# DUBSON0/iterative-closest-point-avmi

Measured on AMD Instinct MI355X. Metric: icp_iterations_per_sec, higher is better.
Workload: dtype f64

## Files before the change

iterative-closest-point-avmi_amd/csrc/prep.hip:

```cpp
#include "prep_common.hpp"

namespace icpmi {

#ifndef PREP_AXIS_STEP
#define PREP_AXIS_STEP 4
#endif
#ifndef ICPMI_PREP_WPS
#define ICPMI_PREP_WPS 6
#endif
constexpr int PREP_THREADS = 512;
constexpr int PREP_MAXW = PREP_THREADS / ICPMI_WAVE;
constexpr int PREP_MAX_POINTS = 4096;

constexpr float PREP_POLAR_Q = 6.283185307179586f / 2097152.0f;
__device__ __forceinline__ uint32_t prep_polar_key21(double x, double y) {
    const float t = (atan2f((float)y, (float)x) + 3.14159265f) * (2097152.0f / 6.283185307179586f);
    const int k = (int)t;
    return (uint32_t)(k < 0 ? 0 : (k > 2097151 ? 2097151 : k));
}
__device__ __forceinline__ float prep_polar_image(uint32_t k21) { return (float)k21 * PREP_POLAR_Q - 3.14159265f; }

template <int E>
__device__ __forceinline__ void prep_sort_polar32(const double* __restrict__ P, int M, uint64_t* keys, uint32_t* rows) {
    uint32_t v[E];
#pragma unroll
    for (int e = 0; e < E; ++e) {
        const int i = e * PREP_THREADS + (int)threadIdx.x;
        v[e] = i < M ? (prep_polar_key21(P[2 * i], P[2 * i + 1]) << 11) | (uint32_t)i : 0xffffffffu;
    }
    bitonic_sort_regs_fixed<uint32_t, E, PREP_THREADS>(v, reinterpret_cast<uint32_t*>(keys));
    __syncthreads();
#pragma unroll
    for (int e = 0; e < E; ++e) {
        const int i = (int)threadIdx.x * E + e;
        rows[i] = v[e] == 0xffffffffu ? 0xffffffffu : (v[e] & 0x7ffu);
        keys[i] = v[e] == 0xffffffffu ? ~0ull : f64_sortable((double)prep_polar_image(v[e] >> 11));
    }
    __syncthreads();
}

template <int E>
__device__ __forceinline__ void prep_sort_regs(const double* __restrict__ P, int M, int dir, uint64_t* by_row, uint64_t* keys,
                                               uint32_t* rows) {
    if (dir == SWEEP_POLAR) { prep_sort_polar32<E>(P, M, keys, rows); return; }
    constexpr uint64_t ROW_MASK = 0x7ff;
    uint64_t v[E];
#pragma unroll
    for (int e = 0; e < E; ++e) {
        const int i = (int)threadIdx.x * E + e;
        const uint64_t k = i < M ? f64_sortable(proj(dir, P[2 * i], P[2 * i + 1])) : ~0ull;
        by_row[i] = k;
        v[e] = i < M ? ((k & ~ROW_MASK) | (uint64_t)i) : ~0ull;
    }
    bitonic_sort_regs_fixed<uint64_t, E, PREP_THREADS>(v, keys);
    int bad = 0;
#pragma unroll
    for (int e = 0; e < E; ++e) {
        const int i = (int)threadIdx.x * E + e;
        const uint32_t r = v[e] == ~0ull ? 0xffffffffu : (uint32_t)(v[e] & ROW_MASK);
        rows[i] = r;
        keys[i] = r == 0xffffffffu ? ~0ull : by_row[r];
    }
    __syncthreads();
#pragma unroll
    for (int e = 0; e < E; ++e) {
        const int i = (int)threadIdx.x * E + e;
        if (i + 1 < M && (keys[i] > keys[i + 1] || (keys[i] == keys[i + 1] && rows[i] > rows[i + 1]))) bad = 1;
    }
    if (__syncthreads_or(bad)) {
        if (threadIdx.x == 0)
            for (int i = 1; i < M; ++i) {
                const uint64_t k = keys[i];
                const uint32_t r = rows[i];
                int j = i - 1;
                while (j >= 0 && (keys[j] > k || (keys[j] == k && rows[j] > r))) { keys[j + 1] = keys[j]; rows[j + 1] = rows[j]; --j; }
                keys[j + 1] = k; rows[j + 1] = r;
            }
        __syncthreads();
    }
}

template <int KK, bool GRID>
__global__ __launch_bounds__(PREP_THREADS, (KK <= 13 ? ICPMI_PREP_WPS : (KK <= 16 ? 4 : 2))) void prep_targets_kernel(
    const double* __restrict__ pts, const int32_t* __restrict__ off, const int32_t* __restrict__ cnt,
    const int32_t* __restrict__ cloud_ids, int k, double2* __restrict__ g_sxy, double2* __restrict__ g_snrm,
    int32_t* __restrict__ g_sorig, float* __restrict__ g_skey, int32_t* __restrict__ g_dir, double* __restrict__ out_normals,
    int lds_points, int split, int polar) {
    extern __shared__ __attribute__((aligned(16))) unsigned char dyn[];
    __shared__ double dsc[8 * PREP_MAXW];
    __shared__ int hist[6 * PREP_BINS];
    const int ci = blockIdx.x / split, part = blockIdx.x % split;
    const int c = cloud_ids ? cloud_ids[ci] : ci;
    const int M = cnt ? cnt[c] : off[c + 1] - off[c];
    if (off[c + 1] - off[c] > PREP_MAX_POINTS) return;
    if (M <= 0 || M > lds_points) { if (threadIdx.x == 0) g_dir[c] = -1; return; }
    const double* P = pts + (size_t)off[c] * 2;
    int npad = 64;
    while (npad < M) npad <<= 1;
    double2* sxy = reinterpret_cast<double2*>(dyn);
    int32_t* sorig = reinterpret_cast<int32_t*>(dyn + (size_t)lds_points * 16);
    float* sth = reinterpret_cast<float*>(dyn + (size_t)lds_points * 20);
    const size_t scratch_at = GRID ? (size_t)lds_points * 24 : 0;
    const bool reg_sort = npad <= 4 * PREP_THREADS;
    const int nsort = reg_sort ? max(npad, PREP_THREADS) : npad;
    uint64_t* by_row = reinterpret_cast<uint64_t*>(dyn + scratch_at);
    uint64_t* keys = reinterpret_cast<uint64_t*>(dyn + scratch_at + (reg_sort ? (size_t)nsort * 8 : 0));
    uint32_t* rows = reinterpret_cast<uint32_t*>(reinterpret_cast<unsigned char*>(keys) + (size_t)nsort * 8);

    double bounds[4];
    const int dir = choose_axis<PREP_THREADS>(P, M, dsc, hist, bounds, polar, (!GRID && M >= 512) ? PREP_AXIS_STEP : 1);
    if (reg_sort) {
        if (nsort == PREP_THREADS) prep_sort_regs<1>(P, M, dir, by_row, keys, rows);
        else if (nsort == 2 * PREP_THREADS) prep_sort_regs<2>(P, M, dir, by_row, keys, rows);
        else prep_sort_regs<4>(P, M, dir, by_row, keys, rows);
    } else {
        for (int i = threadIdx.x; i < npad; i += PREP_THREADS) {
            keys[i] = i < M ? f64_sortable(dir == SWEEP_POLAR ? polar_key(P[2 * i], P[2 * i + 1]) : proj(dir, P[2 * i], P[2 * i + 1])) : ~0ull;
            rows[i] = i < M ? (uint32_t)i : 0xffffffffu;
        }
        __syncthreads();
        bitonic_sort_pairs(keys, rows, npad);
    }
    double2* o_sxy = g_sxy + off[c];
    int32_t* o_sorig = g_sorig + off[c];
    float* o_skey = g_skey + off[c];
    int my_row[PREP_MAX_POINTS / PREP_THREADS];
    float my_key[PREP_MAX_POINTS / PREP_THREADS];
#pragma unroll
    for (int u = 0; u < PREP_MAX_POINTS / PREP_THREADS; ++u) {
        const int i = u * PREP_THREADS + (int)threadIdx.x;
        my_row[u] = i < M ? (int)rows[i] : 0;
        my_key[u] = i < M ? (float)f64_unsortable(keys[i]) : 0.0f;
    }
    __syncthreads();
#pragma unroll
    for (int u = 0; u < PREP_MAX_POINTS / PREP_THREADS; ++u) {
        const int i = u * PREP_THREADS + (int)threadIdx.x;
        if (i < M) {
            const int row = my_row[u];
            const double2 p = make_double2(P[2 * row], P[2 * row + 1]);
            sxy[i] = p; sorig[i] = row;
            if (KK > 0 && !GRID && dir == SWEEP_POLAR) sth[i] = my_key[u];
            if (part == 0) { o_sxy[i] = p; o_sorig[i] = row; o_skey[i] = my_key[u]; }
        }
    }
    if (threadIdx.x == 0 && part == 0) g_dir[c] = dir;
    __syncthreads();
    if constexpr (KK > 0) {
        const int kc = min(k, M - 1);
        const int kk = kc + 1;
        double2* o_snrm = g_snrm + off[c];
        double* o_rows = out_normals ? out_normals + (size_t)off[c] * 2 : nullptr;
        const int per = (M + split - 1) / split;
        if constexpr (GRID) {
            const int cells_cap = min(4096, 2 * npad);
            uint32_t* cell_end = reinterpret_cast<uint32_t*>(dyn + scratch_at);
            uint16_t* cell_pts = reinterpret_cast<uint16_t*>(cell_end + cells_cap);
            const PrepGrid grid = prep_grid_build(sxy, M, bounds, kk, cell_end, cell_pts, cells_cap, hist);
            prep_normals_grid<KK>(sxy, sorig, M, min(M, part * per), min(M, (part + 1) * per), kk, grid, o_snrm, o_rows);
        } else {
            if (dir == SWEEP_POLAR) prep_normals_polar<KK>(sxy, sorig, sth, M, min(M, part * per), min(M, (part + 1) * per), kk, o_snrm, o_rows);
            else prep_normals<KK>(sxy, sorig, M, min(M, part * per), min(M, (part + 1) * per), dir, kk, o_snrm, o_rows);
        }
    }
}


constexpr int ANYK_THREADS = 256;
__device__ __forceinline__ int anyk_lower_bound(const double2* sxy, int M, int dir, double v) {
    int lo = 0, hi = M;
    while (lo < hi) {
        const int mid = (lo + hi) >> 1;
        const double2 c = sxy[mid];
        if (proj(dir, c.x, c.y) < v) lo = mid + 1; else hi = mid;
    }
    return lo;
}
__global__ __launch_bounds__(ANYK_THREADS) void normals_anyk_kernel(
    const int32_t* __restrict__ off, const int32_t* __restrict__ cnt, const int32_t* __restrict__ cloud_ids, int k,
    const double2* __restrict__ g_sxy, double2* __restrict__ g_snrm, const int32_t* __restrict__ g_sorig,
    const int32_t* __restrict__ g_dir, double* __restrict__ out_normals, int sel_cap) {
    extern __shared__ __attribute__((aligned(16))) unsigned char dyn[];
    int32_t* sel = reinterpret_cast<int32_t*>(dyn) + (size_t)wave_id() * sel_cap;
    const int c = cloud_ids ? cloud_ids[blockIdx.y] : blockIdx.y;
    const int M = cnt ? min(cnt[c], off[c + 1] - off[c]) : off[c + 1] - off[c];
    const int dir = g_dir[c];
    if (M <= 0 || dir < 0) return;
    const double2* sxy = g_sxy + off[c];
    const int32_t* sorig = g_sorig + off[c];
    double2* o_snrm = g_snrm + off[c];
    double* o_rows = out_normals ? out_normals + (size_t)off[c] * 2 : nullptr;
    const int kk = min(min(k, M - 1) + 1, sel_cap);
    const int lane = lane_id();
    const int waves = gridDim.x * (ANYK_THREADS / ICPMI_WAVE);
    for (int s = blockIdx.x * (ANYK_THREADS / ICPMI_WAVE) + wave_id(); s < M; s += waves) {
        const double2 q = sxy[s];
        int lo = 0, hi = M;
        if (dir < SWEEP_POLAR) {
            const int a0 = max(0, s - kk), a1 = min(M - 1, s + kk);
            double r2 = 0.0;
            for (int i = a0 + lane; i <= a1; i += ICPMI_WAVE) r2 = fmax(r2, sweep_d2(q.x, q.y, sxy[i]));
            r2 = wave_max(r2);
            if (a1 - a0 + 1 >= kk) {
                const double uq = proj(dir, q.x, q.y);
                const double w = sqrt(r2) * 1.4142135623730951 * 1.000001 + 1e-9 * (1.0 + fabs(uq));
                lo = anyk_lower_bound(sxy, M, dir, uq - w);
                hi = anyk_lower_bound(sxy, M, dir, uq + w + 1e-9 * (1.0 + fabs(uq)));
                hi = min(M, hi + 1);
            }
        }
        double last_d = -1.0;
        int last_row = -1;
        for (int j = 0; j < kk; ++j) {
            double bd = __builtin_inf();
            int brow = 0x7fffffff, bpos = -1;
            for (int i = lo + lane; i < hi; i += ICPMI_WAVE) {
                const double d2 = sweep_d2(q.x, q.y, sxy[i]);
                const int row = sorig[i];
                const bool after = d2 > last_d || (d2 == last_d && row > last_row);
                if (after && (d2 < bd || (d2 == bd && row < brow))) { bd = d2; brow = row; bpos = i; }
            }
#pragma unroll
            for (int o = 32; o > 0; o >>= 1) {
                const double od = __shfl_xor(bd, o, ICPMI_WAVE);
                const int orow = __shfl_xor(brow, o, ICPMI_WAVE), opos = __shfl_xor(bpos, o, ICPMI_WAVE);
                if (od < bd || (od == bd && orow < brow)) { bd = od; brow = orow; bpos = opos; }
            }
            last_d = bd; last_row = brow;
            if (lane == 0) sel[j] = bpos;
        }
        __builtin_amdgcn_fence(__ATOMIC_RELEASE, "workgroup");
        __builtin_amdgcn_wave_barrier();
        __builtin_amdgcn_fence(__ATOMIC_ACQUIRE, "workgroup");
        if (lane == 0) {
            double mx = 0.0, my = 0.0;
            for (int j = 0; j < kk; ++j) { const double2 p = sxy[sel[j]]; mx += p.x; my += p.y; }
            mx /= (double)kk; my /= (double)kk;
            double sxx = 0.0, sxy_ = 0.0, syy = 0.0;
            for (int j = 0; j < kk; ++j) {
                const double2 p = sxy[sel[j]];
                const double dx = p.x - mx, dy = p.y - my;
                sxx += dx * dx; sxy_ += dx * dy; syy += dy * dy;
            }
            double vx = 1.0, vy = 0.0;
            if (kk > 1) {
                const double den = (double)(kk - 1);
                smallest_evec_2x2(sxx / den, sxy_ / den, syy / den, vx, vy);
            }
            double nn = sqrt(vx * vx + vy * vy);
            nn = nn < 1e-10 ? 1e-10 : nn;
            const double2 n2 = make_double2(vx / nn, vy / nn);
            o_snrm[s] = n2;
            if (o_rows) { const int row = sorig[s]; o_rows[2 * row] = n2.x; o_rows[2 * row + 1] = n2.y; }
        }
        __builtin_amdgcn_wave_barrier();
    }
}

using PrepKernel = void (*)(const double*, const int32_t*, const int32_t*, const int32_t*, int, double2*, double2*, int32_t*,
                            float*, int32_t*, double*, int, int, int);
struct PrepChoice {
    PrepKernel kernel;
    int kk;
    bool grid;
};
template <int KK>
static PrepChoice prep_choice_of(bool use_grid) {
    if (use_grid && KK > 0) return {prep_targets_kernel<KK, true>, KK, true};
    return {prep_targets_kernel<KK, false>, KK, false};
}
static PrepChoice prep_choice(int normal_k, bool use_grid) {
    if (normal_k > 31) return {prep_targets_kernel<0, false>, 0, false};
    if (normal_k < 0) return prep_choice_of<0>(use_grid);
    if (normal_k + 1 <= 6) return prep_choice_of<6>(use_grid);
    if (normal_k + 1 <= 8) return prep_choice_of<8>(use_grid);
    if (normal_k + 1 <= 11) return prep_choice_of<11>(use_grid);
    if (normal_k + 1 <= 13) return prep_choice_of<13>(use_grid);
    if (normal_k + 1 <= 16) return prep_choice_of<16>(use_grid);
    return prep_choice_of<32>(use_grid);
}

}

extern "C" size_t icpmi_prepared_bytes(int32_t total_rows, int32_t n_clouds, int32_t max_n) {
    if (total_rows < 0 || n_clouds < 0 || max_n < 0) return 0;
    return icpmi::PreparedView(nullptr, total_rows, n_clouds).core_bytes +
           (max_n > icpmi::PREP_MAX_POINTS ? icpmi::prep_big_scratch_bytes(max_n) : 0);
}

extern "C" int icpmi_prepare_targets(const double* pts, const int32_t* off_dev, const int32_t* off_host,
                                     const int32_t* cnt_dev, const int32_t* cloud_ids, const int32_t* cloud_ids_host,
                                     int32_t n_sel, int32_t n_clouds, int32_t total_rows, int32_t max_n,
                                     int32_t normal_k, double* out_normals, void* prepared, size_t prepared_bytes,
                                     void* stream) {
    return icpmi_prepare_targets_ex(pts, off_dev, off_host, cnt_dev, cloud_ids, cloud_ids_host, n_sel, n_clouds, total_rows, max_n,
                                    normal_k, out_normals, prepared, prepared_bytes, 0, stream);
}

extern "C" int icpmi_prepare_targets_ex(const double* pts, const int32_t* off_dev, const int32_t* off_host,
                                        const int32_t* cnt_dev, const int32_t* cloud_ids, const int32_t* cloud_ids_host,
                                        int32_t n_sel, int32_t n_clouds, int32_t total_rows, int32_t max_n,
                                        int32_t normal_k, double* out_normals, void* prepared, size_t prepared_bytes,
                                        int32_t allow_polar, void* stream) {
    using namespace icpmi;
    if (!pts || !off_dev || !prepared || n_sel < 0 || n_clouds < 0 || total_rows < 0 || max_n < 0) return ICPMI_ERR_ARG;
    if (normal_k > 31 && (size_t)(normal_k + 1) * 4 * (ANYK_THREADS / ICPMI_WAVE) > 96 * 1024) return ICPMI_ERR_UNSUPPORTED;
    if (prepared_bytes < icpmi_prepared_bytes(total_rows, n_clouds, max_n)) return ICPMI_ERR_WORKSPACE;
    if (max_n > PREP_MAX_POINTS && !off_host) return ICPMI_ERR_ARG;
    if (cloud_ids && max_n > PREP_MAX_POINTS && !cloud_ids_host) return ICPMI_ERR_ARG;
    if (n_sel == 0 || max_n == 0) return ICPMI_OK;
    hipStream_t st = (hipStream_t)stream;
    const PreparedView v(prepared, total_rows, n_clouds);
    int small_max = max_n;
    if (max_n > PREP_MAX_POINTS) {
        void* scratch = (unsigned char*)prepared + v.core_bytes;
        const size_t scratch_bytes = prepared_bytes - v.core_bytes;
        small_max = 0;
        for (int i = 0; i < n_sel; ++i) {
            const int c = cloud_ids ? cloud_ids_host[i] : i;
            if (c < 0 || c >= n_clouds) return ICPMI_ERR_ARG;
            const int n = off_host[c + 1] - off_host[c];
            if (n <= PREP_MAX_POINTS) { small_max = n > small_max ? n : small_max; continue; }
            const size_t o = (size_t)off_host[c];
            const int rc = prep_big_cloud(pts + o * 2, cnt_dev ? cnt_dev + c : nullptr, n, normal_k > 31 ? -1 : normal_k, v.sxy + o, v.snrm + o,
                                          v.sorig + o, v.dir + c, out_normals ? out_normals + o * 2 : nullptr, scratch,
                                          scratch_bytes, st);
            if (rc != ICPMI_OK) return rc;
        }
        if (small_max == 0 && normal_k <= 31) return ICPMI_OK;
    }
    int npad = 64;
    while (npad < small_max) npad <<= 1;
    const int lds_points = (small_max + 63) / 64 * 64;
    const size_t sort_bytes = npad <= 4 * PREP_THREADS ? (size_t)(npad > PREP_THREADS ? npad : PREP_THREADS) * 20 : (size_t)npad * 12;
    const size_t lds_sep = (size_t)lds_points * 24 + sort_bytes;
    const size_t lds_alias = (size_t)lds_points * 24 > sort_bytes ? (size_t)lds_points * 24 : sort_bytes;
    int polar = allow_polar && max_n <= 2048 ? 1 : 0;
    if (const char* env = option("POLAR")) polar = polar ? (env[0] == '0' ? 0 : (env[0] == '2' ? 2 : 1)) : 0;
    int split = 256 / n_sel;
    split = split < 1 ? 1 : (split > 16 ? 16 : split);
    int use_grid = split > 1 && !polar;
    if (const char* env = option("PREP_KNN")) use_grid = env[0] == 'g' ? 1 : (env[0] == 's' ? 0 : use_grid);
    const PrepChoice pc = prep_choice(normal_k, use_grid);
    if (small_max > 0) {
        const size_t lds = pc.grid ? lds_sep : lds_alias;
        const int parts = pc.kk > 0 ? split : 1;
        if (dyn_lds((const void*)pc.kernel, lds) != hipSuccess) return ICPMI_ERR_HIP;
        pc.kernel<<<n_sel * parts, PREP_THREADS, lds, st>>>(pts, off_dev, cnt_dev, cloud_ids, normal_k, v.sxy, v.snrm, v.sorig, v.skey,
                                                            v.dir, out_normals, lds_points, parts, polar);
    }
    if (normal_k > 31) {
        ICPMI_LAUNCH_CHECK();
        const int kcap = normal_k + 1 < max_n ? normal_k + 1 : max_n;
        const int sel_cap = (kcap + 63) / 64 * 64;
        const size_t lds_k = (size_t)sel_cap * 4 * (ANYK_THREADS / ICPMI_WAVE);
        if (dyn_lds((const void*)normals_anyk_kernel, lds_k) != hipSuccess) return ICPMI_ERR_HIP;
        int per_cloud = 2048 / n_sel;
        per_cloud = per_cloud < 1 ? 1 : (per_cloud > 256 ? 256 : per_cloud);
        normals_anyk_kernel<<<dim3(per_cloud, n_sel), ANYK_THREADS, lds_k, st>>>(off_dev, cnt_dev, cloud_ids, normal_k, v.sxy, v.snrm, v.sorig,
                                                                                  v.dir, out_normals, sel_cap);
    }
    ICPMI_LAUNCH_CHECK();
    return ICPMI_OK;
}
```

iterative-closest-point-avmi_amd/csrc/prep_common.hpp:

```cpp
#pragma once
#include "linalg.hpp"
#include "sort.hpp"
#include "sweep.hpp"

namespace icpmi {

struct PreparedView {
    double2 *sxy, *snrm;
    int32_t* sorig;
    float* skey;
    int32_t* dir;
    size_t core_bytes;
    PreparedView(const void* prepared, int32_t total_rows, int32_t n_clouds = 0) {
        unsigned char* const b = (unsigned char*)prepared;
        const auto at = [b](size_t o) { return b ? b + o : nullptr; };
        sxy = (double2*)b;
        snrm = (double2*)at((size_t)total_rows * 16);
        sorig = (int32_t*)at((size_t)total_rows * 32);
        skey = (float*)at((size_t)total_rows * 36);
        dir = (int32_t*)at((size_t)total_rows * 40);
        core_bytes = align256((size_t)total_rows * 40 + (size_t)n_clouds * 4) + 256;
    }
};

inline hipError_t prepared_relayout(const PreparedView& src, const PreparedView& dst, size_t rows, size_t clouds, size_t dst_clouds,
                                    hipStream_t st) {
    const auto copy = [st](void* d, const void* s, size_t bytes) {
        return bytes ? hipMemcpyAsync(d, s, bytes, hipMemcpyDeviceToDevice, st) : hipSuccess;
    };
    hipError_t e = copy(dst.sxy, src.sxy, rows * sizeof(double2));
    if (e == hipSuccess) e = copy(dst.snrm, src.snrm, rows * sizeof(double2));
    if (e == hipSuccess) e = copy(dst.sorig, src.sorig, rows * sizeof(int32_t));
    if (e == hipSuccess) e = copy(dst.skey, src.skey, rows * sizeof(float));
    if (e == hipSuccess) e = copy(dst.dir, src.dir, clouds * sizeof(int32_t));
    if (e == hipSuccess && dst_clouds > clouds) e = hipMemsetAsync(dst.dir + clouds, 0xFF, (dst_clouds - clouds) * sizeof(int32_t), st);
    return e;
}

size_t prep_big_scratch_bytes(int n);
int prep_big_cloud(const double* P, const int32_t* cnt_c, int n_cap, int normal_k, double2* o_sxy, double2* o_snrm,
                   int32_t* o_sorig, int32_t* dir_c, double* o_rows, void* scratch, size_t scratch_bytes, hipStream_t st);

constexpr int PREP_BINS = 64;

template <int THREADS>
__device__ __forceinline__ int choose_axis(const double* __restrict__ P, int M, double* dsc, int* hist, double* bounds = nullptr,
                                           int polar = 0, int step = 1) {
    constexpr int MAXW = THREADS / ICPMI_WAVE;
    double mn[4], mx[4];
#pragma unroll
    for (int d = 0; d < 4; ++d) { mn[d] = __builtin_inf(); mx[d] = -__builtin_inf(); }
    for (int i = threadIdx.x * step; i < M; i += THREADS * step) {
        const double x = P[2 * i], y = P[2 * i + 1];
#pragma unroll
        for (int d = 0; d < 4; ++d) { const double u = proj(d, x, y); mn[d] = fmin(mn[d], u); mx[d] = fmax(mx[d], u); }
    }
    const int w = wave_id(), l = lane_id();
#pragma unroll
    for (int d = 0; d < 4; ++d) { mn[d] = wave_min(mn[d]); mx[d] = wave_max(mx[d]); }
    if (l == 0)
#pragma unroll
        for (int d = 0; d < 4; ++d) { dsc[d * MAXW + w] = mn[d]; dsc[(4 + d) * MAXW + w] = mx[d]; }
    for (int i = threadIdx.x; i < (polar ? 6 : 4) * PREP_BINS; i += THREADS) hist[i] = 0;
    __syncthreads();
#pragma unroll
    for (int d = 0; d < 4; ++d) {
        double a = __builtin_inf(), b = -__builtin_inf();
        for (int q = 0; q < MAXW; ++q) { a = fmin(a, dsc[d * MAXW + q]); b = fmax(b, dsc[(4 + d) * MAXW + q]); }
        mn[d] = a; mx[d] = b;
    }
    double scale[4];
#pragma unroll
    for (int d = 0; d < 4; ++d) { const double r = mx[d] - mn[d]; scale[d] = r > 0.0 ? (double)PREP_BINS / r : 0.0; }
    for (int i = threadIdx.x * step; i < M; i += THREADS * step) {
        const double x = P[2 * i], y = P[2 * i + 1];
#pragma unroll
        for (int d = 0; d < 4; ++d) {
            int b = (int)((proj(d, x, y) - mn[d]) * scale[d]);
            b = b < 0 ? 0 : (b >= PREP_BINS ? PREP_BINS - 1 : b);
            atomicAdd(&hist[d * PREP_BINS + b], 1);
        }
        if (polar) {
            const float xf = (float)x, yf = (float)y;
            int b = (int)((atan2f(yf, xf) + 3.14159265f) * (PREP_BINS / 6.2831853f));
            b = b < 0 ? 0 : (b >= PREP_BINS ? PREP_BINS - 1 : b);
            const float r = __builtin_amdgcn_sqrtf(xf * xf + yf * yf);
            const float w = r > 1e-3f ? 1.0f / r : 1e3f;
            atomicAdd(&hist[4 * PREP_BINS + b], 1);
            atomicAdd(reinterpret_cast<unsigned int*>(&hist[5 * PREP_BINS + b]), (unsigned int)(w * 1024.0f));
        }
    }
    __syncthreads();
    if (bounds) { bounds[0] = mn[0]; bounds[1] = mx[0]; bounds[2] = mn[1]; bounds[3] = mx[1]; }
    static_assert(PREP_BINS == ICPMI_WAVE, "one lane per bin");
    int dir = 0;
    double bestc = __builtin_inf();
#pragma unroll
    for (int d = 0; d < 4; ++d) {
        const double cn = (double)hist[d * PREP_BINS + l];
        const double s = wave_sum(cn * cn);
        const double r = mx[d] - mn[d];
        const double cost = r > 0.0 ? (d < 2 ? 1.0 : 1.4142135623730951) * s / r : __builtin_inf();
        if (cost < bestc) { bestc = cost; dir = d; }
    }
    if (polar) {
        const double s = wave_sum((double)hist[4 * PREP_BINS + l] * ((double)(unsigned int)hist[5 * PREP_BINS + l] * (1.0 / 1024.0)));
        if (s * (1.0 / 6.283185307179586) < bestc || polar == 2) dir = SWEEP_POLAR;
    }
    return dir;
}

template <int N>
struct SortNet {
    int n;
    int a[N * 8], b[N * 8];
};
template <int N>
constexpr SortNet<N> make_sortnet() {
    SortNet<N> r{};
    int P = 1;
    while (P < N) P <<= 1;
    for (int p = 1; p < P; p <<= 1)
        for (int k = p; k >= 1; k >>= 1)
            for (int j = k % p; j <= P - 1 - k; j += 2 * k)
                for (int i = 0; i <= (k - 1 < P - j - k - 1 ? k - 1 : P - j - k - 1); ++i)
                    if ((i + j) / (p * 2) == (i + j + k) / (p * 2) && i + j + k < N) {
                        r.a[r.n] = i + j; r.b[r.n] = i + j + k; ++r.n;
                    }
    return r;
}

template <int KK>
struct TopKP {
    double d[KK];
    int p[KK];
    template <int I>
    __device__ __forceinline__ void init_from() {
        if constexpr (I < KK) { d[I] = __builtin_inf(); p[I] = 0; init_from<I + 1>(); }
    }
    __device__ __forceinline__ void init() { init_from<0>(); }
    template <int I>
    __device__ __forceinline__ void load_from(const double2* sxy, int b0, const double2 q) {
        if constexpr (I < KK) {
            const double2 c = sxy[b0 + I];
            const double dx = q.x - c.x, dy = q.y - c.y;
            double s = 0.0;
            s += dx * dx;
            s += dy * dy;
            d[I] = s; p[I] = b0 + I;
            load_from<I + 1>(sxy, b0, q);
        }
    }
    static constexpr SortNet<KK> NET = make_sortnet<KK>();
    template <int C>
    __device__ __forceinline__ void net_from(const int32_t* sorig) {
        if constexpr (C < NET.n) {
            constexpr int A = NET.a[C], B = NET.b[C];
            bool sw = d[B] < d[A];
            if (d[B] == d[A]) sw = sorig[p[B]] < sorig[p[A]];
            const double da = d[A], db = d[B];
            const int pa = p[A], pb = p[B];
            d[A] = sw ? db : da; d[B] = sw ? da : db;
            p[A] = sw ? pb : pa; p[B] = sw ? pa : pb;
            net_from<C + 1>(sorig);
        }
    }
    __device__ __forceinline__ void init_block(const double2* sxy, const int32_t* sorig, int b0, const double2 q) {
        load_from<0>(sxy, b0, q);
        net_from<0>(sorig);
    }
    template <int I>
    __device__ __forceinline__ void bubble(const int32_t* sorig) {
        if constexpr (I > 0) {
            if (d[I] < d[I - 1] || (d[I] == d[I - 1] && sorig[p[I]] < sorig[p[I - 1]])) {
                const double td = d[I - 1]; const int tp = p[I - 1];
                d[I - 1] = d[I]; p[I - 1] = p[I];
                d[I] = td; p[I] = tp;
                bubble<I - 1>(sorig);
            }
        }
    }
    __device__ __forceinline__ bool push(double s, int pos, const int32_t* sorig) {
        if (s < d[KK - 1] || (s == d[KK - 1] && sorig[pos] < sorig[p[KK - 1]])) {
            d[KK - 1] = s; p[KK - 1] = pos;
            bubble<KK - 1>(sorig);
            return true;
        }
        return false;
    }
    template <int I>
    __device__ __forceinline__ double kth_from(int k, double v) const {
        if constexpr (I < KK) return kth_from<I + 1>(k, I == k ? d[I] : v);
        else return v;
    }
    __device__ __forceinline__ double kth(int k) const { return kth_from<1>(k, d[0]); }
    template <int I, typename F>
    __device__ __forceinline__ void for_first(int kk, F&& f) const {
        if constexpr (I < KK) {
            if (I < kk) f(p[I]);
            for_first<I + 1>(kk, f);
        }
    }
};

template <int KK>
__device__ __forceinline__ void emit_normal(const TopKP<KK>& top, int kk, const double2* sxy, const int32_t* sorig, int s,
                                            double2* __restrict__ out_sorted, double* __restrict__ out_rows) {
    double mx = 0.0, my = 0.0;
    top.template for_first<0>(kk, [&](int pos) { const double2 c = sxy[pos]; mx += c.x; my += c.y; });
    mx /= (double)kk; my /= (double)kk;
    double sxx = 0.0, sxy_ = 0.0, syy = 0.0;
    top.template for_first<0>(kk, [&](int pos) {
        const double2 c = sxy[pos];
        const double dx = c.x - mx, dy = c.y - my;
        sxx += dx * dx; sxy_ += dx * dy; syy += dy * dy;
    });
    double vx = 1.0, vy = 0.0;
    if (kk > 1) {
        const double den = (double)(kk - 1);
        smallest_evec_2x2(sxx / den, sxy_ / den, syy / den, vx, vy);
    }
    double nn = sqrt(vx * vx + vy * vy);
    nn = nn < 1e-10 ? 1e-10 : nn;
    const double2 n2 = make_double2(vx / nn, vy / nn);
    out_sorted[s] = n2;
    if (out_rows) { const int row = sorig[s]; out_rows[2 * row] = n2.x; out_rows[2 * row + 1] = n2.y; }
}

template <int KK>
__device__ __forceinline__ void prep_normals(const double2* sxy, const int32_t* sorig, int M, int s_begin, int s_end, int dir, int kk,
                                             double2* __restrict__ out_sorted, double* __restrict__ out_rows) {
    const double2 c_lo = sxy[0], c_hi = sxy[M - 1];
    const double uabs = fmax(fabs(proj(dir, c_lo.x, c_lo.y)), fabs(proj(dir, c_hi.x, c_hi.y)));
    const double pa = dir == 1 ? 0.0 : 1.0, pb = dir == 0 ? 0.0 : (dir == 3 ? -1.0 : 1.0);
    for (int s = s_begin + threadIdx.x; s < s_end; s += blockDim.x) {
        const double2 q = sxy[s];
        const double uq = q.x * pa + q.y * pb;
        TopKP<KK> top;
        double bound = __builtin_inf();
        const double eps = dir < 2 ? 0.0 : 4.5e-16 * (fabs(uq) + uabs);
        const double widen = dir < 2 ? 1.0 : 2.000000000000002;
        int lo, hi;
        if (M >= KK) {
            const int b0 = min(max(s - KK / 2, 0), M - KK);
            top.init_block(sxy, sorig, b0, q);
            bound = (kk == KK ? top.d[KK - 1] : top.kth(kk - 1)) * widen;
            lo = b0 - 1; hi = b0 + KK;
        } else {
            top.init();
            top.push(0.0, s, sorig);
            lo = s - 1; hi = s + 1;
        }
        double2 cr = sweep_load(sxy, hi, M), cl = sweep_load(sxy, lo, M);
        while (lo >= 0 || hi < M) {
            const double2 nr = sweep_load(sxy, hi + 1, M), nl = sweep_load(sxy, lo - 1, M);
            const double gr = (cr.x * pa + cr.y * pb) - uq - eps, gl = uq - (cl.x * pa + cl.y * pb) - eps;
            const bool inr = hi < M && !(gr > 0.0 && gr * gr > bound);
            const bool inl = lo >= 0 && !(gl > 0.0 && gl * gl > bound);
            const double sr = sweep_d2(q.x, q.y, cr), sl = sweep_d2(q.x, q.y, cl);
            bool changed = false;
            if (inr) changed = top.push(sr, hi, sorig);
            if (inl) changed = top.push(sl, lo, sorig) || changed;
            if (changed) bound = (kk == KK ? top.d[KK - 1] : top.kth(kk - 1)) * widen;
            hi = inr ? hi + 1 : M;
            lo = inl ? lo - 1 : -1;
            cr = nr; cl = nl;
        }
        emit_normal<KK>(top, kk, sxy, sorig, s, out_sorted, out_rows);
    }
}

template <int KK>
__device__ __forceinline__ void prep_normals_polar(const double2* sxy, const int32_t* sorig, const float* sth, int M, int s_begin, int s_end,
                                                   int kk, double2* __restrict__ out_sorted, double* __restrict__ out_rows) {
    for (int s = s_begin + threadIdx.x; s < s_end; s += blockDim.x) {
        const double2 q = sxy[s];
        const float thq = sth[s];
        const float kw = 1.00001f / __builtin_amdgcn_sqrtf((float)(q.x * q.x + q.y * q.y));
        TopKP<KK> top;
        float W = __builtin_inff();
        auto window = [&](double kth) {
            const float t = (__builtin_amdgcn_sqrtf((float)kth) * 1.000001f + 1e-18f) * kw;
            W = t <= 0.7f ? (t + 0.3f * t * t * t) * 1.000001f + 1.6e-5f : __builtin_inff();
        };
        int lo, hi, remaining;
        if (M >= KK) {
            const int b0 = min(max(s - KK / 2, 0), M - KK);
            top.init_block(sxy, sorig, b0, q);
            window(kk == KK ? top.d[KK - 1] : top.kth(kk - 1));
            lo = b0 - 1; hi = b0 + KK; remaining = M - KK;
        } else {
            top.init();
            top.push(0.0, s, sorig);
            lo = s - 1; hi = s + 1; remaining = M - 1;
        }
        float offr = 0.0f, offl = 0.0f;
        if (hi >= M) { hi -= M; offr = 6.2831855f; }
        if (lo < 0) { lo += M; offl = 6.2831855f; }
        bool openr = true, openl = true;
        float tr = sth[hi], tl = sth[lo];
        double2 cr = sxy[hi], cl = sxy[lo];
        while ((openr || openl) && remaining > 0) {
            const int nh = hi + 1 == M ? 0 : hi + 1, nl = lo == 0 ? M - 1 : lo - 1;
            const float ntr = sth[nh], ntl = sth[nl];
            const double2 ncr = sxy[nh], ncl = sxy[nl];
            const bool inr = openr && !((tr + offr) - thq > W);
            bool inl = openl && !(thq - (tl - offl) > W);
            if (inr && inl && remaining == 1) inl = false;
            const double sr = sweep_d2(q.x, q.y, cr), sl = sweep_d2(q.x, q.y, cl);
            bool changed = false;
            if (inr) changed = top.push(sr, hi, sorig);
            if (inl) changed = top.push(sl, lo, sorig) || changed;
            if (changed) window(kk == KK ? top.d[KK - 1] : top.kth(kk - 1));
            openr = inr; openl = inl;
            remaining -= (inr ? 1 : 0) + (inl ? 1 : 0);
            if (inr) { if (nh == 0) offr = 6.2831855f; hi = nh; tr = ntr; cr = ncr; }
            if (inl) { if (lo == 0) offl = 6.2831855f; lo = nl; tl = ntl; cl = ncl; }
        }
        emit_normal<KK>(top, kk, sxy, sorig, s, out_sorted, out_rows);
    }
}

struct PrepGrid {
    double min_x, min_y, h;
    int nx, ny;
    const uint32_t* cell_end;
    const uint16_t* cell_pts;
};

__device__ __forceinline__ int grid_cell_1d(double v, double mn, double h, int n) {
    const int c = (int)floor((v - mn) / h);
    return c < 0 ? 0 : (c >= n ? n - 1 : c);
}

__device__ __forceinline__ PrepGrid prep_grid_build(const double2* sxy, int M, const double* bounds, int kk, uint32_t* cell_end,
                                                    uint16_t* cell_pts, int cells_cap, int* wave_tot) {
    PrepGrid g;
    g.min_x = bounds[0]; g.min_y = bounds[2];
    const double w = bounds[1] - bounds[0], hg = bounds[3] - bounds[2];
    double h = 0.55 * (double)kk * 2.0 * (w + hg) / (double)M;
    if (!(h > 0.0) || !(h < 1e300)) h = 1.0;
    int nx, ny;
    for (;;) {
        const double fx = floor(w / h) + 1.0, fy = floor(hg / h) + 1.0;
        if (fx * fy <= (double)cells_cap) { nx = (int)fx; ny = (int)fy; break; }
        h *= 1.3;
    }
    g.h = h; g.nx = nx; g.ny = ny;
    g.cell_end = cell_end; g.cell_pts = cell_pts;
    const int nc = nx * ny;
    for (int c = threadIdx.x; c < nc; c += blockDim.x) cell_end[c] = 0;
    __syncthreads();
    for (int i = threadIdx.x; i < M; i += blockDim.x) {
        const double2 p = sxy[i];
        atomicAdd(&cell_end[grid_cell_1d(p.y, g.min_y, h, ny) * nx + grid_cell_1d(p.x, g.min_x, h, nx)], 1u);
    }
    __syncthreads();
    {
        const int per = (nc + (int)blockDim.x - 1) / (int)blockDim.x;
        const int lo = min(nc, (int)threadIdx.x * per), hi = min(nc, lo + per);
        uint32_t sum = 0;
        for (int c = lo; c < hi; ++c) sum += cell_end[c];
        uint32_t inc = sum;
#pragma unroll
        for (int o = 1; o < ICPMI_WAVE; o <<= 1) {
            const uint32_t t = (uint32_t)__shfl_up((int)inc, o, ICPMI_WAVE);
            if (lane_id() >= o) inc += t;
        }
        if (lane_id() == ICPMI_WAVE - 1) wave_tot[wave_id()] = (int)inc;
        __syncthreads();
        uint32_t run = inc - sum;
        for (int w = 0; w < wave_id(); ++w) run += (uint32_t)wave_tot[w];
        for (int c = lo; c < hi; ++c) { const uint32_t n = cell_end[c]; cell_end[c] = run; run += n; }
    }
    __syncthreads();
    for (int i = threadIdx.x; i < M; i += blockDim.x) {
        const double2 p = sxy[i];
        const uint32_t slot = atomicAdd(&cell_end[grid_cell_1d(p.y, g.min_y, h, ny) * nx + grid_cell_1d(p.x, g.min_x, h, nx)], 1u);
        cell_pts[slot] = (uint16_t)i;
    }
    __syncthreads();
    return g;
}

template <int KK>
__device__ __forceinline__ void prep_normals_grid(const double2* sxy, const int32_t* sorig, int M, int s_begin, int s_end, int kk,
                                                  const PrepGrid g, double2* __restrict__ out_sorted, double* __restrict__ out_rows) {
    for (int s = s_begin + threadIdx.x; s < s_end; s += blockDim.x) {
        const double2 q = sxy[s];
        TopKP<KK> top;
        top.init();
        const int cx = grid_cell_1d(q.x, g.min_x, g.h, g.nx), cy = grid_cell_1d(q.y, g.min_y, g.h, g.ny);
        const int kmax = max(max(cx, g.nx - 1 - cx), max(cy, g.ny - 1 - cy));
        for (int k = 0; k <= kmax; ++k) {
            const int n_row = k == 0 ? 1 : 2 * (2 * k + 1), n_ring = k == 0 ? 1 : 8 * k;
            for (int idx = 0; idx < n_ring; ++idx) {
                int xx, yy;
                if (idx < n_row) { xx = cx - k + (idx >> 1); yy = (idx & 1) ? cy + k : cy - k; }
                else { const int j = idx - n_row; yy = cy - k + 1 + (j >> 1); xx = (j & 1) ? cx + k : cx - k; }
                if (xx < 0 || xx >= g.nx || yy < 0 || yy >= g.ny) continue;
                const int c = yy * g.nx + xx;
                const uint32_t e = g.cell_end[c];
                for (uint32_t t = c ? g.cell_end[c - 1] : 0u; t < e; ++t) {
                    const int i = g.cell_pts[t];
                    const double2 p = sxy[i];
                    const double dx = q.x - p.x, dy = q.y - p.y;
                    double d2 = 0.0;
                    d2 += dx * dx;
                    d2 += dy * dy;
                    top.push(d2, i, sorig);
                }
            }
            const double kth = kk == KK ? top.d[KK - 1] : top.kth(kk - 1);
            const double reach = (double)k * g.h;
            if (kth < reach * reach * 0.999999999) break;
        }
        emit_normal<KK>(top, kk, sxy, sorig, s, out_sorted, out_rows);
    }
}

}
```

Baseline: 42.09 million.

## Load prep points into registers once and share them across axis choice and sort

The prep kernel now loads each thread's x/y points (and polar bearings) into registers once. Those register values feed both the axis-selection histogram and the register bitonic sort, replacing separate global re-reads and duplicate atan2 calls. Axis choice is generalized over a sample source and gains a DPP-based cross-wave min/max reduction. Only wave 0 computes the direction and broadcasts it through shared memory, and one barrier in the polar sort is dropped. The polar sort row mapping changes from strided to blocked, and register pressure rises with E.

```diff
diff --git a/iterative-closest-point-avmi_amd/csrc/prep.hip b/iterative-closest-point-avmi_amd/csrc/prep.hip
--- a/iterative-closest-point-avmi_amd/csrc/prep.hip
+++ b/iterative-closest-point-avmi_amd/csrc/prep.hip
@@ -13,42 +13,44 @@
 constexpr int PREP_MAX_POINTS = 4096;
 
 constexpr float PREP_POLAR_Q = 6.283185307179586f / 2097152.0f;
-__device__ __forceinline__ uint32_t prep_polar_key21(double x, double y) {
-    const float t = (atan2f((float)y, (float)x) + 3.14159265f) * (2097152.0f / 6.283185307179586f);
+__device__ __forceinline__ uint32_t prep_polar_key21(float th) {
+    const float t = (th + 3.14159265f) * (2097152.0f / 6.283185307179586f);
     const int k = (int)t;
     return (uint32_t)(k < 0 ? 0 : (k > 2097151 ? 2097151 : k));
 }
 __device__ __forceinline__ float prep_polar_image(uint32_t k21) { return (float)k21 * PREP_POLAR_Q - 3.14159265f; }
 
 template <int E>
-__device__ __forceinline__ void prep_sort_polar32(const double* __restrict__ P, int M, uint64_t* keys, uint32_t* rows) {
+__device__ __forceinline__ int prep_row(int e) { return (int)threadIdx.x * E + e; }
+
+template <int E>
+__device__ __forceinline__ void prep_sort_polar32(const float (&th)[E], int M, uint64_t* keys, uint32_t* rows) {
     uint32_t v[E];
 #pragma unroll
     for (int e = 0; e < E; ++e) {
-        const int i = e * PREP_THREADS + (int)threadIdx.x;
-        v[e] = i < M ? (prep_polar_key21(P[2 * i], P[2 * i + 1]) << 11) | (uint32_t)i : 0xffffffffu;
+        const int i = prep_row<E>(e);
+        v[e] = i < M ? (prep_polar_key21(th[e]) << 11) | (uint32_t)i : 0xffffffffu;
     }
     bitonic_sort_regs_fixed<uint32_t, E, PREP_THREADS>(v, reinterpret_cast<uint32_t*>(keys));
+#pragma unroll
+    for (int e = 0; e < E; ++e) {
+        const int i = (int)threadIdx.x * E + e;
+        rows[i] = i >= M ? 0xffffffffu : (v[e] & 0x7ffu);
+        keys[i] = i >= M ? ~0ull : f64_sortable((double)prep_polar_image(v[e] >> 11));
+    }
     __syncthreads();
-#pragma unroll
-    for (int e = 0; e < E; ++e) {
-        const int i = (int)threadIdx.x * E + e;
-        rows[i] = v[e] == 0xffffffffu ? 0xffffffffu : (v[e] & 0x7ffu);
-        keys[i] = v[e] == 0xffffffffu ? ~0ull : f64_sortable((double)prep_polar_image(v[e] >> 11));
-    }
-    __syncthreads();
 }
 
 template <int E>
-__device__ __forceinline__ void prep_sort_regs(const double* __restrict__ P, int M, int dir, uint64_t* by_row, uint64_t* keys,
-                                               uint32_t* rows) {
-    if (dir == SWEEP_POLAR) { prep_sort_polar32<E>(P, M, keys, rows); return; }
+__device__ __forceinline__ void prep_sort_regs(const double (&x)[E], const double (&y)[E], const float (&th)[E], int M, int dir,
+                                               uint64_t* by_row, uint64_t* keys, uint32_t* rows) {
+    if (dir == SWEEP_POLAR) { prep_sort_polar32<E>(th, M, keys, rows); return; }
     constexpr uint64_t ROW_MASK = 0x7ff;
     uint64_t v[E];
 #pragma unroll
     for (int e = 0; e < E; ++e) {
-        const int i = (int)threadIdx.x * E + e;
-        const uint64_t k = i < M ? f64_sortable(proj(dir, P[2 * i], P[2 * i + 1])) : ~0ull;
+        const int i = prep_row<E>(e);
+        const uint64_t k = i < M ? f64_sortable(proj(dir, x[e], y[e])) : ~0ull;
         by_row[i] = k;
         v[e] = i < M ? ((k & ~ROW_MASK) | (uint64_t)i) : ~0ull;
     }
@@ -78,6 +80,27 @@
             }
         __syncthreads();
     }
+}
+
+template <int E>
+__device__ __forceinline__ int prep_axis_and_sort(const double* __restrict__ P, int M, double* dsc, int* hist, double* bounds, int polar,
+                                                  int step, uint64_t* by_row, uint64_t* keys, uint32_t* rows) {
+    double x[E], y[E];
+    float th[E];
+#pragma unroll
+    for (int e = 0; e < E; ++e) {
+        const int i = prep_row<E>(e);
+        x[e] = i < M ? P[2 * i] : 0.0;
+        y[e] = i < M ? P[2 * i + 1] : 0.0;
+    }
+#pragma unroll
+    for (int e = 0; e < E; ++e) {
+        th[e] = 0.0f;
+        if (polar && prep_row<E>(e) < M) th[e] = atan2f((float)y[e], (float)x[e]);
+    }
+    const int dir = choose_axis_on<PREP_THREADS>(AxisSampleRegs<E, PREP_AXIS_STEP>{x, y, th, M, step == 1}, dsc, hist, bounds, polar);
+    prep_sort_regs<E>(x, y, th, M, dir, by_row, keys, rows);
+    return dir;
 }
 
 template <int KK, bool GRID>
@@ -108,12 +131,14 @@
     uint32_t* rows = reinterpret_cast<uint32_t*>(reinterpret_cast<unsigned char*>(keys) + (size_t)nsort * 8);
 
     double bounds[4];
-    const int dir = choose_axis<PREP_THREADS>(P, M, dsc, hist, bounds, polar, (!GRID && M >= 512) ? PREP_AXIS_STEP : 1);
+    const int step = (!GRID && M >= 512) ? PREP_AXIS_STEP : 1;
+    int dir;
     if (reg_sort) {
-        if (nsort == PREP_THREADS) prep_sort_regs<1>(P, M, dir, by_row, keys, rows);
-        else if (nsort == 2 * PREP_THREADS) prep_sort_regs<2>(P, M, dir, by_row, keys, rows);
-        else prep_sort_regs<4>(P, M, dir, by_row, keys, rows);
+        if (nsort == PREP_THREADS) dir = prep_axis_and_sort<1>(P, M, dsc, hist, GRID ? bounds : nullptr, polar, step, by_row, keys, rows);
+        else if (nsort == 2 * PREP_THREADS) dir = prep_axis_and_sort<2>(P, M, dsc, hist, GRID ? bounds : nullptr, polar, step, by_row, keys, rows);
+        else dir = prep_axis_and_sort<4>(P, M, dsc, hist, GRID ? bounds : nullptr, polar, step, by_row, keys, rows);
     } else {
+        dir = choose_axis<PREP_THREADS>(P, M, dsc, hist, GRID ? bounds : nullptr, polar, step);
         for (int i = threadIdx.x; i < npad; i += PREP_THREADS) {
             keys[i] = i < M ? f64_sortable(dir == SWEEP_POLAR ? polar_key(P[2 * i], P[2 * i + 1]) : proj(dir, P[2 * i], P[2 * i + 1])) : ~0ull;
             rows[i] = i < M ? (uint32_t)i : 0xffffffffu;
diff --git a/iterative-closest-point-avmi_amd/csrc/prep_common.hpp b/iterative-closest-point-avmi_amd/csrc/prep_common.hpp
--- a/iterative-closest-point-avmi_amd/csrc/prep_common.hpp
+++ b/iterative-closest-point-avmi_amd/csrc/prep_common.hpp
@@ -44,70 +44,126 @@
 constexpr int PREP_BINS = 64;
 
 template <int THREADS>
+struct AxisSampleGlobal {
+    const double* __restrict__ P;
+    int M, step;
+    __device__ __forceinline__ bool any() const { return (int)threadIdx.x * step < M; }
+    template <typename F>
+    __device__ __forceinline__ void for_each(bool bearing, F&& f) const {
+        for (int i = threadIdx.x * step; i < M; i += THREADS * step) {
+            const double x = P[2 * i], y = P[2 * i + 1];
+            f(x, y, bearing ? atan2f((float)y, (float)x) : 0.0f);
+        }
+    }
+};
+template <int E, int STEP>
+struct AxisSampleRegs {
+    const double (&x)[E];
+    const double (&y)[E];
+    const float (&th)[E];
+    int M;
+    bool every;
+    static __device__ __forceinline__ int row(int e) { return (int)threadIdx.x * E + e; }
+    __device__ __forceinline__ bool any() const {
+        bool a = false;
+#pragma unroll
+        for (int e = 0; e < E; ++e) a = a || (row(e) < M && (every || row(e) % STEP == 0));
+        return a;
+    }
+    template <typename F>
+    __device__ __forceinline__ void for_each(bool, F&& f) const {
+#pragma unroll
+        for (int e = 0; e < E; ++e)
+            if (row(e) < M && (every || row(e) % STEP == 0)) f(x[e], y[e], th[e]);
+    }
+};
+
+template <int THREADS, typename Sample>
+__device__ __forceinline__ int choose_axis_on(const Sample& pts, double* dsc, int* hist, double* bounds = nullptr, int polar = 0) {
+    constexpr int MAXW = THREADS / ICPMI_WAVE;
+    for (int i = threadIdx.x; i < (polar ? 6 : 4) * PREP_BINS; i += THREADS) hist[i] = 0;
+    double mn[4], mx[4];
+#pragma unroll
+    for (int d = 0; d < 4; ++d) { mn[d] = __builtin_inf(); mx[d] = -__builtin_inf(); }
+    pts.for_each(false, [&](double x, double y, float) {
+#pragma unroll
+        for (int d = 0; d < 4; ++d) { const double u = proj(d, x, y); mn[d] = fmin(mn[d], u); mx[d] = fmax(mx[d], u); }
+    });
+    const int w = wave_id(), l = lane_id();
+#pragma unroll
+    for (int d = 0; d < 4; ++d) { mn[d] = wave_min(mn[d]); mx[d] = wave_max(mx[d]); }
+    if (l == 0)
+#pragma unroll
+        for (int d = 0; d < 4; ++d) { dsc[d * MAXW + w] = mn[d]; dsc[(4 + d) * MAXW + w] = mx[d]; }
+    __syncthreads();
+    if (bounds || w == 0 || __any(pts.any())) {
+        if constexpr (MAXW == 8) {
+            double v = l < 32 ? dsc[l] : -dsc[l];
+            v = fmin(v, dpp_f64<0xB1>(v));
+            v = fmin(v, dpp_f64<0x4E>(v));
+            v = fmin(v, dpp_f64<0x141>(v));
+#pragma unroll
+            for (int d = 0; d < 4; ++d) { mn[d] = readlane_f64(v, d * 8); mx[d] = -readlane_f64(v, 32 + d * 8); }
+        } else {
+#pragma unroll
+            for (int d = 0; d < 4; ++d) {
+                double a = __builtin_inf(), b = -__builtin_inf();
+                for (int q = 0; q < MAXW; ++q) { a = fmin(a, dsc[d * MAXW + q]); b = fmax(b, dsc[(4 + d) * MAXW + q]); }
+                mn[d] = a; mx[d] = b;
+            }
+        }
+    }
+    if (pts.any()) {
+        double scale[4];
+#pragma unroll
+        for (int d = 0; d < 4; ++d) { const double r = mx[d] - mn[d]; scale[d] = r > 0.0 ? (double)PREP_BINS / r : 0.0; }
+        pts.for_each(polar != 0, [&](double x, double y, float th) {
+#pragma unroll
+            for (int d = 0; d < 4; ++d) {
+                int b = (int)((proj(d, x, y) - mn[d]) * scale[d]);
+                b = b < 0 ? 0 : (b >= PREP_BINS ? PREP_BINS - 1 : b);
+                atomicAdd(&hist[d * PREP_BINS + b], 1);
+            }
+            if (polar) {
+                const float xf = (float)x, yf = (float)y;
+                int b = (int)((th + 3.14159265f) * (PREP_BINS / 6.2831853f));
+                b = b < 0 ? 0 : (b >= PREP_BINS ? PREP_BINS - 1 : b);
+                const float r = __builtin_amdgcn_sqrtf(xf * xf + yf * yf);
+                const float w = r > 1e-3f ? 1.0f / r : 1e3f;
+                atomicAdd(&hist[4 * PREP_BINS + b], 1);
+                atomicAdd(reinterpret_cast<unsigned int*>(&hist[5 * PREP_BINS + b]), (unsigned int)(w * 1024.0f));
+            }
+        });
+    }
+    __syncthreads();
+    if (bounds) { bounds[0] = mn[0]; bounds[1] = mx[0]; bounds[2] = mn[1]; bounds[3] = mx[1]; }
+    static_assert(PREP_BINS == ICPMI_WAVE, "one lane per bin");
+    int* const answer = reinterpret_cast<int*>(dsc);
+    if (w == 0) {
+        int dir = 0;
+        double bestc = __builtin_inf();
+#pragma unroll
+        for (int d = 0; d < 4; ++d) {
+            const double cn = (double)hist[d * PREP_BINS + l];
+            const double s = wave_sum(cn * cn);
+            const double r = mx[d] - mn[d];
+            const double cost = r > 0.0 ? (d < 2 ? 1.0 : 1.4142135623730951) * s / r : __builtin_inf();
+            if (cost < bestc) { bestc = cost; dir = d; }
+        }
+        if (polar) {
+            const double s = wave_sum((double)hist[4 * PREP_BINS + l] * ((double)(unsigned int)hist[5 * PREP_BINS + l] * (1.0 / 1024.0)));
+            if (s * (1.0 / 6.283185307179586) < bestc || polar == 2) dir = SWEEP_POLAR;
+        }
+        if (l == 0) *answer = dir;
+    }
+    __syncthreads();
+    return *answer;
+}
+
+template <int THREADS>
 __device__ __forceinline__ int choose_axis(const double* __restrict__ P, int M, double* dsc, int* hist, double* bounds = nullptr,
                                            int polar = 0, int step = 1) {
-    constexpr int MAXW = THREADS / ICPMI_WAVE;
-    double mn[4], mx[4];
-#pragma unroll
-    for (int d = 0; d < 4; ++d) { mn[d] = __builtin_inf(); mx[d] = -__builtin_inf(); }
-    for (int i = threadIdx.x * step; i < M; i += THREADS * step) {
-        const double x = P[2 * i], y = P[2 * i + 1];
-#pragma unroll
-        for (int d = 0; d < 4; ++d) { const double u = proj(d, x, y); mn[d] = fmin(mn[d], u); mx[d] = fmax(mx[d], u); }
-    }
-    const int w = wave_id(), l = lane_id();
-#pragma unroll
-    for (int d = 0; d < 4; ++d) { mn[d] = wave_min(mn[d]); mx[d] = wave_max(mx[d]); }
-    if (l == 0)
-#pragma unroll
-        for (int d = 0; d < 4; ++d) { dsc[d * MAXW + w] = mn[d]; dsc[(4 + d) * MAXW + w] = mx[d]; }
-    for (int i = threadIdx.x; i < (polar ? 6 : 4) * PREP_BINS; i += THREADS) hist[i] = 0;
-    __syncthreads();
-#pragma unroll
-    for (int d = 0; d < 4; ++d) {
-        double a = __builtin_inf(), b = -__builtin_inf();
-        for (int q = 0; q < MAXW; ++q) { a = fmin(a, dsc[d * MAXW + q]); b = fmax(b, dsc[(4 + d) * MAXW + q]); }
-        mn[d] = a; mx[d] = b;
-    }
-    double scale[4];
-#pragma unroll
-    for (int d = 0; d < 4; ++d) { const double r = mx[d] - mn[d]; scale[d] = r > 0.0 ? (double)PREP_BINS / r : 0.0; }
-    for (int i = threadIdx.x * step; i < M; i += THREADS * step) {
-        const double x = P[2 * i], y = P[2 * i + 1];
-#pragma unroll
-        for (int d = 0; d < 4; ++d) {
-            int b = (int)((proj(d, x, y) - mn[d]) * scale[d]);
-            b = b < 0 ? 0 : (b >= PREP_BINS ? PREP_BINS - 1 : b);
-            atomicAdd(&hist[d * PREP_BINS + b], 1);
-        }
-        if (polar) {
-            const float xf = (float)x, yf = (float)y;
-            int b = (int)((atan2f(yf, xf) + 3.14159265f) * (PREP_BINS / 6.2831853f));
-            b = b < 0 ? 0 : (b >= PREP_BINS ? PREP_BINS - 1 : b);
-            const float r = __builtin_amdgcn_sqrtf(xf * xf + yf * yf);
-            const float w = r > 1e-3f ? 1.0f / r : 1e3f;
-            atomicAdd(&hist[4 * PREP_BINS + b], 1);
-            atomicAdd(reinterpret_cast<unsigned int*>(&hist[5 * PREP_BINS + b]), (unsigned int)(w * 1024.0f));
-        }
-    }
-    __syncthreads();
-    if (bounds) { bounds[0] = mn[0]; bounds[1] = mx[0]; bounds[2] = mn[1]; bounds[3] = mx[1]; }
-    static_assert(PREP_BINS == ICPMI_WAVE, "one lane per bin");
-    int dir = 0;
-    double bestc = __builtin_inf();
-#pragma unroll
-    for (int d = 0; d < 4; ++d) {
-        const double cn = (double)hist[d * PREP_BINS + l];
-        const double s = wave_sum(cn * cn);
-        const double r = mx[d] - mn[d];
-        const double cost = r > 0.0 ? (d < 2 ? 1.0 : 1.4142135623730951) * s / r : __builtin_inf();
-        if (cost < bestc) { bestc = cost; dir = d; }
-    }
-    if (polar) {
-        const double s = wave_sum((double)hist[4 * PREP_BINS + l] * ((double)(unsigned int)hist[5 * PREP_BINS + l] * (1.0 / 1024.0)));
-        if (s * (1.0 / 6.283185307179586) < bestc || polar == 2) dir = SWEEP_POLAR;
-    }
-    return dir;
+    return choose_axis_on<THREADS>(AxisSampleGlobal<THREADS>{P, M, step}, dsc, hist, bounds, polar);
 }
 
 template <int N>
```

New measurement: 42.44 million, median of 6. No clear change (+0.8%).
